# praateekmahajan/moving-mnist-vae

Measured on AMD Instinct MI355X. Metric: frames/sec/GPU VAE train step, 20×64×64 batch; ELBO vs CPU ref, higher is better.
Workload: dtype bf16; 1 GPU; BASELINE configs[1]: 256 clips x 20 frames x 64x64 per GPU per step (=5120 frames), conv-VAE z=128, Gaussian NLL sigma=0.1 + KL (normal_vae_1_kl_0_mmd), Adam, random-init weights, Bernoulli(0.0521) q=2 labels; parallelism=dp1, rccl_ranks=1, grad_exchange=none, bn=per-rank batch statistics

## Files before the change

moving-mnist-vae_amd/csrc/conv_fstream.hip:

```cpp
#include <hip/hip_runtime.h>

#include <stdlib.h>
#include <string.h>

#include "kernels.hpp"
#include "tile_common.hpp"

namespace mmvae {

struct Conv3StreamArgs {
  const void* x; const void* w; const void* wsc; void* y; void* ysc;
  const float* pro_scale; const float* pro_shift; int pro_relu;
  float* stats; float* stats_sc;
  const void* ym; const float* ms; const float* mb;
  int N, Ho, Hi;
  int HS, nunits;
};

template <int S, bool SC, bool PRO, bool BS = false>
__global__ __launch_bounds__(256, 2) void conv3_stream_kernel(Conv3StreamArgs a) {
  static_assert(!BS || (S == 1 && !SC && !PRO), "backward sums: the stride-1 data gradient");
  constexpr int KS = 3, PAD = 1, WO = 16, WI = S * WO, CB = 64;
  constexpr int WL = WI + 2;
  constexpr int ROWB = WL * CB;
  constexpr int NSLOT = KS + S;
  constexpr int WAVE_LDS = NSLOT * ROWB;
  constexpr int RV = S * WI * CB / 1024;
  constexpr int NPRIME = (KS - S + S - 1) / S;
  extern __shared__ __attribute__((aligned(16))) char smem[];
  const int t = threadIdx.x, lane = t & 63, wv = __builtin_amdgcn_readfirstlane(t >> 6), gq = lane >> 4, r = lane & 15;
  char* ring = smem + 2048 + wv * WAVE_LDS;
  for (int s = 0; s < NSLOT; ++s) {
    if (lane < 4) *reinterpret_cast<Vec16*>(ring + s * ROWB + lane * 16) = Vec16{{0, 0, 0, 0}};
    else if (lane < 8) *reinterpret_cast<Vec16*>(ring + s * ROWB + (WL - 1) * CB + (lane - 4) * 16) = Vec16{{0, 0, 0, 0}};
  }
  Vec16 wA[KS * KS][2], wS[2];
#pragma unroll
  for (int m = 0; m < 2; ++m) {
    const int c = 8 * (r >> 2) + 4 * m + (r & 3);
#pragma unroll
    for (int tap = 0; tap < KS * KS; ++tap)
      wA[tap][m] = *reinterpret_cast<const Vec16*>(reinterpret_cast<const char*>(a.w) + ((c * KS * KS + tap) * 32 + 8 * gq) * 2);
    wS[m] = SC ? *reinterpret_cast<const Vec16*>(reinterpret_cast<const char*>(a.wsc) + (c * 32 + 8 * gq) * 2) : Vec16{{0, 0, 0, 0}};
  }
  float psc[8], psh[8];
  if (PRO) {
    const int c = (lane & 3) * 8;
#pragma unroll
    for (int j = 0; j < 8; ++j) { psc[j] = a.pro_scale[c + j]; psh[j] = a.pro_shift[c + j]; }
  }
  const float lo = a.pro_relu ? 0.f : -__builtin_inff();
  float bms[8], bmb[8];
  if (BS) {
#pragma unroll
    for (int j = 0; j < 8; ++j) { bms[j] = a.ms[8 * gq + j]; bmb[j] = a.mb[8 * gq + j]; }
  }
  Vec16 yv = Vec16{{0, 0, 0, 0}};
  float st[SC ? 4 : 2][8];
#pragma unroll
  for (int q = 0; q < (SC ? 4 : 2); ++q)
#pragma unroll
    for (int j = 0; j < 8; ++j) st[q][j] = 0.f;

  const bf16_t* __restrict__ X = reinterpret_cast<const bf16_t*>(a.x);
  const int nblk = gridDim.x;
  int u_first, u_step, u_end;
  if ((nblk & 7) == 0) {
    const int per = (a.nunits + 7) >> 3;
    const int lo_u = (blockIdx.x & 7) * per;
    u_first = lo_u + (blockIdx.x >> 3) * 4 + wv; u_step = (nblk >> 3) * 4; u_end = min(a.nunits, lo_u + per);
  } else { u_first = blockIdx.x * 4 + wv; u_step = nblk * 4; u_end = a.nunits; }
  const int nstrips = a.Ho / a.HS;
  const int nq = a.HS + NPRIME;

  Vec16 xv[RV];
  auto issue = [&](int u, int q) {
    const int n = u / nstrips, oh0 = (u - n * nstrips) * a.HS;
    const int top = S * (oh0 + q - NPRIME) + 1;
#pragma unroll
    for (int k = 0; k < RV; ++k) {
      const int byte = (lane + 64 * k) * 16;
      const int rr = byte / (WI * CB), off = byte - rr * (WI * CB);
      const int row = top - S + 1 + rr;
      xv[k] = Vec16{{0, 0, 0, 0}};
      if (row >= 0 && row < a.Hi) xv[k] = *reinterpret_cast<const Vec16*>(reinterpret_cast<const char*>(X) + (((long)n * a.Hi + row) * WI) * CB + off);
    }
    if (BS && q >= NPRIME)
      yv = *reinterpret_cast<const Vec16*>(reinterpret_cast<const char*>(a.ym) + ((((long)n * a.Ho + oh0 + q - NPRIME) * WO + r) * 32 + 8 * gq) * 2);
  };
  auto commit = [&](int u, int q) {
    const int n = u / nstrips, oh0 = (u - n * nstrips) * a.HS;
    const int top = S * (oh0 + q - NPRIME) + 1;
#pragma unroll
    for (int k = 0; k < RV; ++k) {
      const int byte = (lane + 64 * k) * 16;
      const int rr = byte / (WI * CB), off = byte - rr * (WI * CB);
      const int row = top - S + 1 + rr;
      Vec16 v = xv[k];
      if (PRO && row >= 0 && row < a.Hi) {
        float f[8];
        Elem<bf16_t>::unpack(v, f);
#pragma unroll
        for (int j = 0; j < 8; ++j) f[j] = fmaxf(f[j] * psc[j] + psh[j], lo);
        v = Elem<bf16_t>::pack(f);
      }
      *reinterpret_cast<Vec16*>(ring + ((row + 4 * NSLOT) % NSLOT) * ROWB + CB + off) = v;
    }
    (void)n;
  };

  int u = u_first, q = 0;
  if (u < u_end) issue(u, 0);
  while (u < u_end) {
    commit(u, q);
    const Vec16 ycur = yv;
    int un = u, qn = q + 1;
    if (qn == nq) { un = u + u_step; qn = 0; }
    if (un < u_end) issue(un, qn);
    __builtin_amdgcn_sched_barrier(0);
    if (q >= NPRIME) {
      const int n = u / nstrips, oh = (u - n * nstrips) * a.HS + q - NPRIME;
      const int first = S * oh - PAD;
      f32x4 acc[2], asc[2];
#pragma unroll
      for (int m = 0; m < 2; ++m) { acc[m] = (f32x4){0, 0, 0, 0}; asc[m] = (f32x4){0, 0, 0, 0}; }
#pragma unroll
      for (int kh = 0; kh < KS; ++kh) {
        const char* rowp = ring + ((first + kh + 4 * NSLOT) % NSLOT) * ROWB;
#pragma unroll
        for (int kw = 0; kw < KS; ++kw) {
          const Vec16 b = *reinterpret_cast<const Vec16*>(rowp + (S * r + kw) * CB + gq * 16);
          acc[0] = mma_bf16(wA[kh * KS + kw][0], b, acc[0]);
          acc[1] = mma_bf16(wA[kh * KS + kw][1], b, acc[1]);
          if (SC && kh == 1 && kw == 1) { asc[0] = mma_bf16(wS[0], b, asc[0]); asc[1] = mma_bf16(wS[1], b, asc[1]); }
        }
      }
      const long po = (((long)n * a.Ho + oh) * WO + r) * 32 + 8 * gq;
      {
        const float v[8] = {acc[0][0], acc[0][1], acc[0][2], acc[0][3], acc[1][0], acc[1][1], acc[1][2], acc[1][3]};
        if constexpr (BS) {
          float ym[8], vr[8];
          Elem<bf16_t>::unpack(ycur, ym);
          Elem<bf16_t>::unpack(Elem<bf16_t>::pack(v), vr);
#pragma unroll
          for (int j = 0; j < 8; ++j) {
            const float g = (ym[j] * bms[j] + bmb[j] > 0.f) ? vr[j] : 0.f;
            st[0][j] += g; st[1][j] += g * ym[j];
          }
        } else {
#pragma unroll
          for (int j = 0; j < 8; ++j) { st[0][j] += v[j]; st[1][j] += v[j] * v[j]; }
        }
        dstore8<bf16_t>(reinterpret_cast<bf16_t*>(a.y) + po, v, false);
      }
      if constexpr (SC) {
        const float v[8] = {asc[0][0], asc[0][1], asc[0][2], asc[0][3], asc[1][0], asc[1][1], asc[1][2], asc[1][3]};
#pragma unroll
        for (int j = 0; j < 8; ++j) { st[2][j] += v[j]; st[3][j] += v[j] * v[j]; }
        dstore8<bf16_t>(reinterpret_cast<bf16_t*>(a.ysc) + po, v, false);
      }
    }
    __builtin_amdgcn_sched_barrier(0);
    u = un; q = qn;
  }
  float* sb = reinterpret_cast<float*>(smem);
#pragma unroll
  for (int qq = 0; qq < (SC ? 4 : 2); ++qq)
#pragma unroll
    for (int j = 0; j < 8; ++j) {
      const float v = row16_sum(st[qq][j]);
      if (r == 0) sb[wv * 128 + qq * 32 + 8 * gq + j] = v;
    }
  __syncthreads();
  if (t < (SC ? 128 : 64)) {
    const float v = (sb[t] + sb[128 + t]) + (sb[256 + t] + sb[384 + t]);
    float* dst = t < 64 ? a.stats : a.stats_sc;
    if (dst) dst[(long)blockIdx.x * 64 + (t & 63)] = v;
  }
}

bool conv3_stream_ok(int dt, int Cin, int Cout, int k, int s, int p, int Hin, int Win) {
  return dt == DT_BF16 && Cin == 32 && Cout == 32 && k == 3 && p == 1 && (s == 1 || s == 2) && Hin == Win && Win == 16 * s;
}

int launch_conv3_stream(int dt, int stride, const void* x, const void* w, const void* wsc, void* y, void* ysc, const float* pro_scale,
                        const float* pro_shift, int pro_relu, float* stats, float* stats_sc, int N, int Ho, hipStream_t s) {
  if (dt != DT_BF16 || (stride != 1 && stride != 2) || (wsc && stride != 2) || ((wsc != nullptr) != (ysc != nullptr))) {
    set_error("conv3_stream: bf16, stride 1 or 2, shortcut only with stride 2"); return MMVAE_ERR_UNSUPPORTED;
  }
  Conv3StreamArgs a; memset(&a, 0, sizeof(a));
  a.x = x; a.w = w; a.wsc = wsc; a.y = y; a.ysc = ysc; a.pro_scale = pro_scale; a.pro_shift = pro_shift; a.pro_relu = pro_relu;
  a.stats = stats; a.stats_sc = stats_sc; a.N = N; a.Ho = Ho; a.Hi = stride * Ho;
  a.HS = Ho % 8 == 0 ? 8 : Ho;
  a.nunits = N * (Ho / a.HS);
  int gx = stride == 1 ? 768 : 512;
  while (gx > 8 && (long)gx * 4 > a.nunits) gx -= 8;
  const bool pro = pro_scale != nullptr;
  const size_t lds = 2048 + 4 * (size_t)((3 + stride) * (stride * 16 + 2) * 64);
#define MMVAE_C3(S_, SC_, P_) hipLaunchKernelGGL((conv3_stream_kernel<S_, SC_, P_>), dim3(gx), dim3(256), lds, s, a)
  if (stride == 2) { if (wsc) { if (pro) MMVAE_C3(2, true, true); else MMVAE_C3(2, true, false); } else { if (pro) MMVAE_C3(2, false, true); else MMVAE_C3(2, false, false); } }
  else { if (pro) MMVAE_C3(1, false, true); else MMVAE_C3(1, false, false); }
#undef MMVAE_C3
  note_launch_bytes((double)N * 32 * 2.0 * ((double)a.Hi * a.Hi + (double)Ho * Ho * (wsc ? 2 : 1)));
  const int rc = check_launch("conv3_stream");
  return rc ? rc : gx;
}

int launch_conv3_stream_bwd(int dt, const void* dy, const void* w_flipped, void* dx, const void* ym, const float* ms, const float* mb, float* sums,
                            int N, int H, hipStream_t s) {
  if (dt != DT_BF16 || H != 16 || !ym || !ms || !mb || !sums) { set_error("conv3_stream_bwd: bf16, 16x16 maps, mask operand and sums required"); return MMVAE_ERR_UNSUPPORTED; }
  Conv3StreamArgs a; memset(&a, 0, sizeof(a));
  a.x = dy; a.w = w_flipped; a.y = dx; a.stats = sums; a.ym = ym; a.ms = ms; a.mb = mb; a.N = N; a.Ho = H; a.Hi = H;
  a.HS = 8; a.nunits = N * (H / a.HS);
  int gx = 768;
  while (gx > 8 && (long)gx * 4 > a.nunits) gx -= 8;
  const size_t lds = 2048 + 4 * (size_t)(4 * 18 * 64);
  hipLaunchKernelGGL((conv3_stream_kernel<1, false, false, true>), dim3(gx), dim3(256), lds, s, a);
  note_launch_bytes((double)N * 32 * 2.0 * 3.0 * H * H);
  const int rc = check_launch("conv3_stream_bwd");
  return rc ? rc : gx;
}

struct TailFwdStreamArgs {
  const void* y2; const void* ys; const float* s2; const float* b2; const float* ss; const float* bs;
  const float* w; const float* bias; float* r_raw; float* stats;
  int N, H, HS, nunits;
};

template <bool F8I>
__global__ __launch_bounds__(256, 2) void tail_fwd_stream_kernel(TailFwdStreamArgs a) {
  constexpr int KS = 3, W = 64, CB = 32;
  constexpr int NC = F8I ? 16 : 8;
  constexpr int WL = W + 2, ROWB = WL * CB, NSLOT = KS + 1, WAVE_LDS = NSLOT * ROWB, NPRIME = 2;
  extern __shared__ __attribute__((aligned(16))) char smem[];
  const int t = threadIdx.x, lane = t & 63, wv = __builtin_amdgcn_readfirstlane(t >> 6), gq = lane >> 4, r = lane & 15;
  char* ring = smem + 64 + wv * WAVE_LDS;
  for (int s = 0; s < NSLOT; ++s) {
    if (lane < 2) *reinterpret_cast<Vec16*>(ring + s * ROWB + lane * 16) = Vec16{{0, 0, 0, 0}};
    else if (lane < 4) *reinterpret_cast<Vec16*>(ring + s * ROWB + (WL - 1) * CB + (lane - 2) * 16) = Vec16{{0, 0, 0, 0}};
  }
  Vec16 wA[2];
  {
    float f0[8], f1[8];
#pragma unroll
    for (int j = 0; j < 8; ++j) {
      const int c = 8 * (gq & 1) + j;
      f0[j] = r < 3 ? a.w[c * 9 + (gq >> 1) * 3 + r] : 0.f;
      f1[j] = (r < 3 && gq < 2) ? a.w[c * 9 + 2 * 3 + r] : 0.f;
    }
    wA[0] = Elem<bf16_t>::pack(f0); wA[1] = Elem<bf16_t>::pack(f1);
  }
  const float bias = a.bias ? a.bias[0] : 0.f;
  float c2s[NC], c2b[NC], css[NC];
  {
    const int c = F8I ? 0 : (lane & 1) * 8;
#pragma unroll
    for (int j = 0; j < NC; ++j) { c2s[j] = a.s2[c + j]; c2b[j] = a.b2[c + j] + a.bs[c + j]; css[j] = a.ss[c + j]; }
  }
  float st1 = 0.f, st2 = 0.f;
  const int nblk = gridDim.x;
  int u_first, u_step, u_end;
  if ((nblk & 7) == 0) {
    const int per = (a.nunits + 7) >> 3;
    const int lo_u = (blockIdx.x & 7) * per;
    u_first = lo_u + (blockIdx.x >> 3) * 4 + wv; u_step = (nblk >> 3) * 4; u_end = min(a.nunits, lo_u + per);
  } else { u_first = blockIdx.x * 4 + wv; u_step = nblk * 4; u_end = a.nunits; }
  const int nstrips = a.H / a.HS;
  const int nq = a.HS + NPRIME;
  Vec16 v2[2], vs[2];
  auto issue = [&](int u, int q) {
    const int n = u / nstrips, oh0 = (u - n * nstrips) * a.HS;
    const int row = oh0 + q - NPRIME + 1;
#pragma unroll
    for (int k = 0; k < (F8I ? 1 : 2); ++k) {
      v2[k] = Vec16{{0, 0, 0, 0}}; vs[k] = Vec16{{0, 0, 0, 0}};
      if (row >= 0 && row < a.H) {
        const long off = (((long)n * a.H + row) * W) * (F8I ? 16 : CB) + (lane + 64 * k) * 16;
        v2[k] = *reinterpret_cast<const Vec16*>(reinterpret_cast<const char*>(a.y2) + off);
        vs[k] = *reinterpret_cast<const Vec16*>(reinterpret_cast<const char*>(a.ys) + off);
      }
    }
  };
  auto commit = [&](int u, int q) {
    const int n = u / nstrips, oh0 = (u - n * nstrips) * a.HS;
    const int row = oh0 + q - NPRIME + 1;
    const bool in = row >= 0 && row < a.H;
    if constexpr (F8I) {
      float f2[16], fs[16];
#pragma unroll
      for (int q4 = 0; q4 < 4; ++q4) { unpack4_fp8(v2[0].w[q4], f2 + 4 * q4); unpack4_fp8(vs[0].w[q4], fs + 4 * q4); }
#pragma unroll
      for (int j = 0; j < 16; ++j) f2[j] = in ? fmaxf(f2[j] * c2s[j] + c2b[j] + fs[j] * css[j], 0.f) : 0.f;
      char* dstp = ring + ((row + 4 * NSLOT) % NSLOT) * ROWB + CB + lane * 32;
      *reinterpret_cast<Vec16*>(dstp) = Elem<bf16_t>::pack(f2);
      *reinterpret_cast<Vec16*>(dstp + 16) = Elem<bf16_t>::pack(f2 + 8);
    } else {
#pragma unroll
      for (int k = 0; k < 2; ++k) {
        float f2[8], fs[8];
        Elem<bf16_t>::unpack(v2[k], f2);
        Elem<bf16_t>::unpack(vs[k], fs);
#pragma unroll
        for (int j = 0; j < 8; ++j) f2[j] = in ? fmaxf(f2[j] * c2s[j] + c2b[j] + fs[j] * css[j], 0.f) : 0.f;
        *reinterpret_cast<Vec16*>(ring + ((row + 4 * NSLOT) % NSLOT) * ROWB + CB + (lane + 64 * k) * 16) = Elem<bf16_t>::pack(f2);
      }
    }
    (void)n;
  };
  int u = u_first, q = 0;
  if (u < u_end) issue(u, 0);
  while (u < u_end) {
    commit(u, q);
    int un = u, qn = q + 1;
    if (qn == nq) { un = u + u_step; qn = 0; }
    if (un < u_end) issue(un, qn);
    __builtin_amdgcn_sched_barrier(0);
    if (q >= NPRIME) {
      const int n = u / nstrips, oh = (u - n * nstrips) * a.HS + q - NPRIME;
      const char* row01 = ring + ((oh - 1 + (gq >> 1) + 4 * NSLOT) % NSLOT) * ROWB;
      const char* row2 = ring + ((oh + 1 + 4 * NSLOT) % NSLOT) * ROWB;
      float d0[4], d1[4], d2[4];
#pragma unroll
      for (int pt = 0; pt < 4; ++pt) {
        const int po = (16 * pt + r + 1) * CB + (gq & 1) * 16;
        f32x4 acc = mma_bf16(wA[0], *reinterpret_cast<const Vec16*>(row01 + po), (f32x4){0, 0, 0, 0});
        acc = mma_bf16(wA[1], *reinterpret_cast<const Vec16*>(row2 + po), acc);
        d0[pt] = acc[0]; d1[pt] = acc[1]; d2[pt] = acc[2];
        asm volatile("" : "+v"(d0[pt]), "+v"(d1[pt]), "+v"(d2[pt]));
      }
      float outv[4];
#pragma unroll
      for (int pt = 0; pt < 4; ++pt) {
        float left = __builtin_bit_cast(float, __builtin_amdgcn_mov_dpp(__builtin_bit_cast(int, d0[pt]), 0x111, 0xf, 0xf, true));
        if (pt > 0) {
          const float pl = __builtin_bit_cast(float, __builtin_amdgcn_mov_dpp(__builtin_bit_cast(int, d0[pt - 1]), 0x121, 0xf, 0xf, true));
          left = r == 0 ? pl : left;
        }
        float right = __builtin_bit_cast(float, __builtin_amdgcn_mov_dpp(__builtin_bit_cast(int, d2[pt]), 0x101, 0xf, 0xf, true));
        if (pt < 3) {
          const float nr = __builtin_bit_cast(float, __builtin_amdgcn_mov_dpp(__builtin_bit_cast(int, d2[pt + 1]), 0x12f, 0xf, 0xf, true));
          right = r == 15 ? nr : right;
        }
        outv[pt] = (left + d1[pt]) + right + bias;
      }
      if (gq == 0) {
        float* orow = a.r_raw + ((long)n * a.H + oh) * W + r;
#pragma unroll
        for (int pt = 0; pt < 4; ++pt) {
          orow[16 * pt] = outv[pt];
          st1 += outv[pt]; st2 += outv[pt] * outv[pt];
        }
      }
    }
    __builtin_amdgcn_sched_barrier(0);
    u = un; q = qn;
  }
  st1 = row16_sum(st1); st2 = row16_sum(st2);
  float* sb = reinterpret_cast<float*>(smem);
  if (lane == 0) { sb[wv * 2] = st1; sb[wv * 2 + 1] = st2; }
  __syncthreads();
  if (a.stats && t < 2) a.stats[(long)blockIdx.x * 2 + t] = (sb[t] + sb[2 + t]) + (sb[4 + t] + sb[6 + t]);
}

struct ConvT4StreamArgs {
  const void* x; const void* w; void* y;
  const float* pro_scale; const float* pro_shift; int pro_relu;
  float* stats;
  int N, Hi, HS, nunits;
};

template <int WIN, bool PRO, bool F8O = false>
__global__ __launch_bounds__(256, 3) void convT4_stream_kernel(ConvT4StreamArgs a) {
  constexpr int CB = 32, WL = WIN + 2, ROWB = WL * CB, NSLOT = 4, NPRIME = 2;
  constexpr int CBO = F8O ? 16 : 32;
  constexpr int OROWB = 2 * WIN * CBO;
  constexpr int WAVE_LDS = NSLOT * ROWB + OROWB;
  constexpr int XV = (WIN * CB + 1023) / 1024;
  constexpr int NPT = WIN / 16;
  extern __shared__ __attribute__((aligned(16))) char smem[];
  const int t = threadIdx.x, lane = t & 63, wv = __builtin_amdgcn_readfirstlane(t >> 6), gq = lane >> 4, r = lane & 15;
  char* ring = smem + 1024 + wv * WAVE_LDS;
  char* orow = ring + NSLOT * ROWB;
  for (int s = 0; s < NSLOT; ++s) {
    if (lane < 2) *reinterpret_cast<Vec16*>(ring + s * ROWB + lane * 16) = Vec16{{0, 0, 0, 0}};
    else if (lane < 4) *reinterpret_cast<Vec16*>(ring + s * ROWB + (WL - 1) * CB + (lane - 2) * 16) = Vec16{{0, 0, 0, 0}};
  }
  Vec16 wA[4][2];
#pragma unroll
  for (int p = 0; p < 4; ++p)
#pragma unroll
    for (int th = 0; th < 2; ++th)
      wA[p][th] = *reinterpret_cast<const Vec16*>(reinterpret_cast<const char*>(a.w) + p * 2048 + r * 128 + th * 64 + gq * 16);
  const int dwl[2] = {(gq >> 1) ? -1 : 0, (gq >> 1) ? 0 : 1};
  float psc[8], psh[8];
  if (PRO) {
    const int c = (lane & 1) * 8;
#pragma unroll
    for (int j = 0; j < 8; ++j) { psc[j] = a.pro_scale[c + j]; psh[j] = a.pro_shift[c + j]; }
  }
  const float lo = a.pro_relu ? 0.f : -__builtin_inff();
  float st1[4] = {0, 0, 0, 0}, st2[4] = {0, 0, 0, 0};
  const int nblk = gridDim.x;
  int u_first, u_step, u_end;
  if ((nblk & 7) == 0) {
    const int per = (a.nunits + 7) >> 3;
    const int lo_u = (blockIdx.x & 7) * per;
    u_first = lo_u + (blockIdx.x >> 3) * 4 + wv; u_step = (nblk >> 3) * 4; u_end = min(a.nunits, lo_u + per);
  } else { u_first = blockIdx.x * 4 + wv; u_step = nblk * 4; u_end = a.nunits; }
  const int nstrips = a.Hi / a.HS;
  const int nq = a.HS + NPRIME;
  const bool xlane = lane * 16 < WIN * CB;
  Vec16 xv = Vec16{{0, 0, 0, 0}};
  auto issue = [&](int u, int q) {
    const int n = u / nstrips, q0 = (u - n * nstrips) * a.HS;
    const int row = q0 + q - NPRIME + 1;
    xv = Vec16{{0, 0, 0, 0}};
    if (xlane && row >= 0 && row < a.Hi) xv = *reinterpret_cast<const Vec16*>(reinterpret_cast<const char*>(a.x) + (((long)n * a.Hi + row) * WIN) * CB + lane * 16);
  };
  auto commit = [&](int u, int q) {
    const int n = u / nstrips, q0 = (u - n * nstrips) * a.HS;
    const int row = q0 + q - NPRIME + 1;
    if (xlane) {
      Vec16 v = xv;
      if (PRO && row >= 0 && row < a.Hi) {
        float f[8];
        Elem<bf16_t>::unpack(v, f);
#pragma unroll
        for (int j = 0; j < 8; ++j) f[j] = fmaxf(f[j] * psc[j] + psh[j], lo);
        v = Elem<bf16_t>::pack(f);
      }
      *reinterpret_cast<Vec16*>(ring + ((row + 4 * NSLOT) % NSLOT) * ROWB + CB + lane * 16) = v;
    }
    (void)n; (void)XV;
  };
  int u = u_first, q = 0;
  if (u < u_end) issue(u, 0);
  while (u < u_end) {
    commit(u, q);
    int un = u, qn = q + 1;
    if (qn == nq) { un = u + u_step; qn = 0; }
    if (un < u_end) issue(un, qn);
    __builtin_amdgcn_sched_barrier(0);
    if (q >= NPRIME) {
      const int n = u / nstrips, iq = (u - n * nstrips) * a.HS + q - NPRIME;
#pragma unroll
      for (int ph = 0; ph < 2; ++ph) {
#pragma unroll
        for (int pw = 0; pw < 2; ++pw) {
          f32x4 acc[NPT];
#pragma unroll
          for (int pt = 0; pt < NPT; ++pt) acc[pt] = (f32x4){0, 0, 0, 0};
#pragma unroll
          for (int th = 0; th < 2; ++th) {
            const int dh = ph == 0 ? (th == 0 ? 0 : -1) : (th == 0 ? 1 : 0);
            const char* rowp = ring + ((iq + dh + 4 * NSLOT) % NSLOT) * ROWB;
#pragma unroll
            for (int pt = 0; pt < NPT; ++pt) {
              const Vec16 b = *reinterpret_cast<const Vec16*>(rowp + (16 * pt + r + dwl[pw] + 1) * CB + (gq & 1) * 16);
              acc[pt] = mma_bf16(wA[2 * ph + pw][th], b, acc[pt]);
            }
          }
#pragma unroll
          for (int pt = 0; pt < NPT; ++pt) {
#pragma unroll
            for (int j = 0; j < 4; ++j) { st1[j] += acc[pt][j]; st2[j] += acc[pt][j] * acc[pt][j]; }
            if constexpr (F8O) {
              *reinterpret_cast<uint32_t*>(orow + (2 * (16 * pt + r) + pw) * CBO + gq * 4) = pack4_fp8(acc[pt][0], acc[pt][1], acc[pt][2], acc[pt][3]);
            } else {
              uint2 o;
              o.x = pack2_bf16(acc[pt][0], acc[pt][1]); o.y = pack2_bf16(acc[pt][2], acc[pt][3]);
              *reinterpret_cast<uint2*>(orow + (2 * (16 * pt + r) + pw) * CB + gq * 8) = o;
            }
          }
        }
        asm volatile("" ::: "memory");
        char* dst = reinterpret_cast<char*>(a.y) + (((long)n * (2 * a.Hi) + 2 * iq + ph) * (2 * WIN)) * CBO;
#pragma unroll
        for (int k = 0; k < OROWB / 1024; ++k) *reinterpret_cast<Vec16*>(dst + (lane + 64 * k) * 16) = *reinterpret_cast<const Vec16*>(orow + (lane + 64 * k) * 16);
      }
    }
    __builtin_amdgcn_sched_barrier(0);
    u = un; q = qn;
  }
  float* sb = reinterpret_cast<float*>(smem);
#pragma unroll
  for (int j = 0; j < 4; ++j) {
    const float v1 = row16_sum(st1[j]), v2 = row16_sum(st2[j]);
    if (r == 0) { sb[wv * 32 + 4 * gq + j] = v1; sb[wv * 32 + 16 + 4 * gq + j] = v2; }
  }
  __syncthreads();
  if (a.stats && t < 32) a.stats[(long)blockIdx.x * 32 + t] = (sb[t] + sb[32 + t]) + (sb[64 + t] + sb[96 + t]);
}

struct Up5TailFwdArgs {
  const void* y1; const float* p1s; const float* p1b; const void* w2;
  const void* xin; const float* pxs; const float* pxb; const void* wu;
  const float* s2; const float* b2; const float* ss; const float* bs;
  const float* w; const float* bias; float* r_raw; float* stats;
  int N, HS, nunits;
};

template <bool PRO_X>
__global__ __launch_bounds__(256, 2) void up5_tail_fwd_kernel(Up5TailFwdArgs a) {
  constexpr int WIN = 32, Hi = 32, W = 64, H = 64, CB = 32;
  constexpr int IWL = WIN + 2, IROWB = IWL * CB, NSLOT = 4;
  constexpr int JWL = W + 2, JROWB = JWL * CB;
  constexpr int WAVE_LDS = 2 * NSLOT * IROWB + NSLOT * JROWB;
  extern __shared__ __attribute__((aligned(16))) char smem[];
  const int t = threadIdx.x, lane = t & 63, wv = __builtin_amdgcn_readfirstlane(t >> 6), gq = lane >> 4, r = lane & 15;
  char* ringA = smem + 64 + wv * WAVE_LDS;
  char* ringX = ringA + NSLOT * IROWB;
  char* ringJ = ringX + NSLOT * IROWB;
  for (int sl = 0; sl < NSLOT; ++sl) {
    if (lane < 2) { *reinterpret_cast<Vec16*>(ringA + sl * IROWB + lane * 16) = Vec16{{0, 0, 0, 0}}; *reinterpret_cast<Vec16*>(ringX + sl * IROWB + lane * 16) = Vec16{{0, 0, 0, 0}}; }
    else if (lane < 4) { *reinterpret_cast<Vec16*>(ringA + sl * IROWB + (IWL - 1) * CB + (lane - 2) * 16) = Vec16{{0, 0, 0, 0}}; *reinterpret_cast<Vec16*>(ringX + sl * IROWB + (IWL - 1) * CB + (lane - 2) * 16) = Vec16{{0, 0, 0, 0}}; }
    else if (lane < 6) *reinterpret_cast<Vec16*>(ringJ + sl * JROWB + (lane - 4) * 16) = Vec16{{0, 0, 0, 0}};
    else if (lane < 8) *reinterpret_cast<Vec16*>(ringJ + sl * JROWB + (JWL - 1) * CB + (lane - 6) * 16) = Vec16{{0, 0, 0, 0}};
  }
  Vec16 w2A[4][2], wuA[4][2];
#pragma unroll
  for (int p = 0; p < 4; ++p)
#pragma unroll
    for (int th = 0; th < 2; ++th) {
      w2A[p][th] = *reinterpret_cast<const Vec16*>(reinterpret_cast<const char*>(a.w2) + p * 2048 + r * 128 + th * 64 + gq * 16);
      wuA[p][th] = *reinterpret_cast<const Vec16*>(reinterpret_cast<const char*>(a.wu) + p * 2048 + r * 128 + th * 64 + gq * 16);
    }
  const int dwl[2] = {(gq >> 1) ? -1 : 0, (gq >> 1) ? 0 : 1};
  Vec16 wT[2];
  {
    float f0[8], f1[8];
#pragma unroll
    for (int j = 0; j < 8; ++j) {
      const int c = 8 * (gq & 1) + j;
      f0[j] = r < 3 ? a.w[c * 9 + (gq >> 1) * 3 + r] : 0.f;
      f1[j] = (r < 3 && gq < 2) ? a.w[c * 9 + 2 * 3 + r] : 0.f;
    }
    wT[0] = Elem<bf16_t>::pack(f0); wT[1] = Elem<bf16_t>::pack(f1);
  }
  const float bias = a.bias ? a.bias[0] : 0.f;
  float p1s[8], p1b[8], pxs[8], pxb[8];
  {
    const int c = (lane & 1) * 8;
#pragma unroll
    for (int j = 0; j < 8; ++j) { p1s[j] = a.p1s[c + j]; p1b[j] = a.p1b[c + j]; pxs[j] = PRO_X ? a.pxs[c + j] : 1.f; pxb[j] = PRO_X ? a.pxb[c + j] : 0.f; }
  }
  float js2[4], jb[4], jss[4];
#pragma unroll
  for (int j = 0; j < 4; ++j) { const int c = 4 * gq + j; js2[j] = a.s2[c]; jb[j] = a.b2[c] + a.bs[c]; jss[j] = a.ss[c]; }
  float st1 = 0.f, st2 = 0.f;
  const int nblk = gridDim.x;
  int u_first, u_step, u_end;
  if ((nblk & 7) == 0) {
    const int per = (a.nunits + 7) >> 3;
    const int lo_u = (blockIdx.x & 7) * per;
    u_first = lo_u + (blockIdx.x >> 3) * 4 + wv; u_step = (nblk >> 3) * 4; u_end = min(a.nunits, lo_u + per);
  } else { u_first = blockIdx.x * 4 + wv; u_step = nblk * 4; u_end = a.nunits; }
  const int nstrips = Hi / a.HS;
  constexpr int NPRIME = 2;
  const int nq = a.HS + 2 + NPRIME;
  Vec16 va = Vec16{{0, 0, 0, 0}}, vx = Vec16{{0, 0, 0, 0}};
  auto issue = [&](int u, int q) {
    const int n = u / nstrips, q0 = (u - n * nstrips) * a.HS;
    const int row = q0 - 1 + q - NPRIME + 1;
    va = Vec16{{0, 0, 0, 0}}; vx = Vec16{{0, 0, 0, 0}};
    if (row >= 0 && row < Hi) {
      const long off = (((long)n * Hi + row) * WIN) * CB + lane * 16;
      va = *reinterpret_cast<const Vec16*>(reinterpret_cast<const char*>(a.y1) + off);
      vx = *reinterpret_cast<const Vec16*>(reinterpret_cast<const char*>(a.xin) + off);
    }
  };
  auto commit = [&](int u, int q) {
    const int n = u / nstrips, q0 = (u - n * nstrips) * a.HS;
    const int row = q0 - 1 + q - NPRIME + 1;
    Vec16 ca = va, cx = vx;
    if (row >= 0 && row < Hi) {
      float f[8];
      Elem<bf16_t>::unpack(ca, f);
#pragma unroll
      for (int j = 0; j < 8; ++j) f[j] = fmaxf(f[j] * p1s[j] + p1b[j], 0.f);
      ca = Elem<bf16_t>::pack(f);
      if (PRO_X) {
        Elem<bf16_t>::unpack(cx, f);
#pragma unroll
        for (int j = 0; j < 8; ++j) f[j] = fmaxf(f[j] * pxs[j] + pxb[j], 0.f);
        cx = Elem<bf16_t>::pack(f);
      }
    }
    const int slot = (row + 4 * NSLOT) % NSLOT;
    *reinterpret_cast<Vec16*>(ringA + slot * IROWB + CB + lane * 16) = ca;
    *reinterpret_cast<Vec16*>(ringX + slot * IROWB + CB + lane * 16) = cx;
    (void)n;
  };
  int u = u_first, q = 0;
  if (u < u_end) issue(u, 0);
  while (u < u_end) {
    commit(u, q);
    int un = u, qn = q + 1;
    if (qn == nq) { un = u + u_step; qn = 0; }
    if (un < u_end) issue(un, qn);
    __builtin_amdgcn_sched_barrier(0);
    if (q >= NPRIME) {
      const int n = u / nstrips, q0 = (u - n * nstrips) * a.HS;
      const int iq = q0 - 1 + q - NPRIME;
      const bool inside = iq >= 0 && iq < Hi;
#pragma unroll
      for (int ph = 0; ph < 2; ++ph) {
        char* jrow = ringJ + ((2 * iq + ph + 8 * NSLOT) % NSLOT) * JROWB;
        if (!inside) {
          for (int i = lane; i < (W * CB) / 16; i += 64) *reinterpret_cast<Vec16*>(jrow + CB + i * 16) = Vec16{{0, 0, 0, 0}};
          continue;
        }
#pragma unroll
        for (int pw = 0; pw < 2; ++pw) {
          f32x4 acc2[2], accS[2];
#pragma unroll
          for (int pt = 0; pt < 2; ++pt) { acc2[pt] = (f32x4){0, 0, 0, 0}; accS[pt] = (f32x4){0, 0, 0, 0}; }
#pragma unroll
          for (int th = 0; th < 2; ++th) {
            const int dh = ph == 0 ? (th == 0 ? 0 : -1) : (th == 0 ? 1 : 0);
            const int sl = (iq + dh + 4 * NSLOT) % NSLOT;
#pragma unroll
            for (int pt = 0; pt < 2; ++pt) {
              const int off = sl * IROWB + (16 * pt + r + dwl[pw] + 1) * CB + (gq & 1) * 16;
              acc2[pt] = mma_bf16(w2A[2 * ph + pw][th], *reinterpret_cast<const Vec16*>(ringA + off), acc2[pt]);
              accS[pt] = mma_bf16(wuA[2 * ph + pw][th], *reinterpret_cast<const Vec16*>(ringX + off), accS[pt]);
            }
          }
#pragma unroll
          for (int pt = 0; pt < 2; ++pt) {
            float o[4];
#pragma unroll
            for (int j = 0; j < 4; ++j) o[j] = fmaxf(acc2[pt][j] * js2[j] + jb[j] + accS[pt][j] * jss[j], 0.f);
            *reinterpret_cast<uint2*>(jrow + (1 + 2 * (16 * pt + r) + pw) * CB + gq * 8) = make_uint2(pack2_bf16(o[0], o[1]), pack2_bf16(o[2], o[3]));
          }
        }
      }
      asm volatile("" ::: "memory");
#pragma unroll
      for (int k = 0; k < 2; ++k) {
        const int oh = 2 * iq - 1 + k;
        if (oh < 2 * q0 || oh >= 2 * (q0 + a.HS) || oh < 0 || oh >= H) continue;
        f32x4 acc[4];
        const char* row01 = ringJ + ((oh - 1 + (gq >> 1) + 8 * NSLOT) % NSLOT) * JROWB;
        const char* row2 = ringJ + ((oh + 1 + 8 * NSLOT) % NSLOT) * JROWB;
#pragma unroll
        for (int pt = 0; pt < 4; ++pt) {
          const int po = (16 * pt + r + 1) * CB + (gq & 1) * 16;
          acc[pt] = mma_bf16(wT[0], *reinterpret_cast<const Vec16*>(row01 + po), (f32x4){0, 0, 0, 0});
          acc[pt] = mma_bf16(wT[1], *reinterpret_cast<const Vec16*>(row2 + po), acc[pt]);
        }
        float d0[4], d1[4], d2[4];
#pragma unroll
        for (int pt = 0; pt < 4; ++pt) {
          d0[pt] = acc[pt][0]; d1[pt] = acc[pt][1]; d2[pt] = acc[pt][2];
          asm volatile("" : "+v"(d0[pt]), "+v"(d1[pt]), "+v"(d2[pt]));
        }
        float outv[4];
#pragma unroll
        for (int pt = 0; pt < 4; ++pt) {
          float left = __builtin_bit_cast(float, __builtin_amdgcn_mov_dpp(__builtin_bit_cast(int, d0[pt]), 0x111, 0xf, 0xf, true));
          if (pt > 0) {
            const float pl = __builtin_bit_cast(float, __builtin_amdgcn_mov_dpp(__builtin_bit_cast(int, d0[pt - 1]), 0x121, 0xf, 0xf, true));
            left = r == 0 ? pl : left;
          }
          float right = __builtin_bit_cast(float, __builtin_amdgcn_mov_dpp(__builtin_bit_cast(int, d2[pt]), 0x101, 0xf, 0xf, true));
          if (pt < 3) {
            const float nr = __builtin_bit_cast(float, __builtin_amdgcn_mov_dpp(__builtin_bit_cast(int, d2[pt + 1]), 0x12f, 0xf, 0xf, true));
            right = r == 15 ? nr : right;
          }
          outv[pt] = (left + d1[pt]) + right + bias;
        }
        if (gq == 0) {
          float* orow = a.r_raw + ((long)n * H + oh) * W + r;
#pragma unroll
          for (int pt = 0; pt < 4; ++pt) {
            orow[16 * pt] = outv[pt];
            st1 += outv[pt]; st2 += outv[pt] * outv[pt];
          }
        }
      }
    }
    __builtin_amdgcn_sched_barrier(0);
    u = un; q = qn;
  }
  st1 = row16_sum(st1); st2 = row16_sum(st2);
  float* sb = reinterpret_cast<float*>(smem);
  if (lane == 0) { sb[wv * 2] = st1; sb[wv * 2 + 1] = st2; }
  __syncthreads();
  if (a.stats && t < 2) a.stats[(long)blockIdx.x * 2 + t] = (sb[t] + sb[2 + t]) + (sb[4 + t] + sb[6 + t]);
}

bool up5_tail_fwd_ok(int dt, int OC, int C, int Cin, int Hin, int Hout) {
  return dt == DT_BF16 && OC == 1 && C == 16 && Cin == 16 && Hin == 32 && Hout == 64;
}
int launch_up5_tail_fwd(const void* y1, const float* p1s, const float* p1b, const void* w2_up, const void* xin, const float* pxs, const float* pxb,
                        const void* wu_up, const float* s2, const float* b2, const float* ss, const float* bs, const float* w, const float* bias,
                        float* r_raw, float* stats, int N, hipStream_t s) {
  Up5TailFwdArgs a; memset(&a, 0, sizeof(a));
  a.y1 = y1; a.p1s = p1s; a.p1b = p1b; a.w2 = w2_up; a.xin = xin; a.pxs = pxs; a.pxb = pxb; a.wu = wu_up;
  a.s2 = s2; a.b2 = b2; a.ss = ss; a.bs = bs; a.w = w; a.bias = bias; a.r_raw = r_raw; a.stats = stats;
  a.N = N; a.HS = 16; a.nunits = N * (32 / a.HS);
  int gx = 512;
  while (gx > 1 && (long)gx * 4 > a.nunits) gx -= gx > 8 ? 8 : 1;
  const size_t lds = 64 + 4 * (size_t)(2 * 4 * 34 * 32 + 4 * 66 * 32);
  static bool attr_set = false;
  if (!attr_set) {
    hipError_t e = hipFuncSetAttribute(reinterpret_cast<const void*>(&up5_tail_fwd_kernel<false>), hipFuncAttributeMaxDynamicSharedMemorySize, 160 * 1024);
    if (e == hipSuccess) e = hipFuncSetAttribute(reinterpret_cast<const void*>(&up5_tail_fwd_kernel<true>), hipFuncAttributeMaxDynamicSharedMemorySize, 160 * 1024);
    if (e != hipSuccess) { set_error("up5_tail_fwd: hipFuncSetAttribute: %s", hipGetErrorString(e)); return MMVAE_ERR_HIP; }
    attr_set = true;
  }
  if (pxs) hipLaunchKernelGGL(up5_tail_fwd_kernel<true>, dim3(gx), dim3(256), lds, s, a);
  else hipLaunchKernelGGL(up5_tail_fwd_kernel<false>, dim3(gx), dim3(256), lds, s, a);
  note_launch_bytes((double)N * (2.0 * 32 * 32 * 16 * 2 + 64 * 64 * 4.0));
  const int rc = check_launch("up5_tail_fwd");
  return rc ? rc : gx;
}

bool convT4_stream_ok(int dt, int Cin, int Cout, int k, int s, int p, int Hin, int Win) {
  return dt == DT_BF16 && Cin == 16 && Cout == 16 && k == 4 && s == 2 && p == 1 && Hin == Win && (Win == 32 || Win == 16);
}
int launch_convT4_stream(int dt, const void* x, const void* w_up, void* y, const float* pro_scale, const float* pro_shift, int pro_relu, float* stats,
                         int N, int Hin, hipStream_t s, int f8out) {
  if (!convT4_stream_ok(dt, 16, 16, 4, 2, 1, Hin, Hin)) { set_error("convT4_stream: bf16, 16 -> 16 channels, k4 s2 p1, 16x16 or 32x32 input"); return MMVAE_ERR_UNSUPPORTED; }
  ConvT4StreamArgs a; memset(&a, 0, sizeof(a));
  a.x = x; a.w = w_up; a.y = y; a.pro_scale = pro_scale; a.pro_shift = pro_shift; a.pro_relu = pro_relu; a.stats = stats;
  a.N = N; a.Hi = Hin; a.HS = Hin % 8 == 0 ? 8 : Hin; a.nunits = N * (Hin / a.HS);
  int gx = Hin == 32 ? 1024 : 768;
  while (gx > 8 && (long)gx * 4 > a.nunits) gx -= 8;
  const bool pro = pro_scale != nullptr;
  const size_t lds = 1024 + 4 * (size_t)(4 * (Hin + 2) * 32 + 2 * Hin * 32);
  if (f8out && Hin != 32) { set_error("convT4_stream: e4m3 output only for the 32x32 -> 64x64 layers"); return MMVAE_ERR_UNSUPPORTED; }
  if (f8out) { if (pro) hipLaunchKernelGGL((convT4_stream_kernel<32, true, true>), dim3(gx), dim3(256), lds, s, a); else hipLaunchKernelGGL((convT4_stream_kernel<32, false, true>), dim3(gx), dim3(256), lds, s, a); }
  else if (Hin == 32) { if (pro) hipLaunchKernelGGL((convT4_stream_kernel<32, true>), dim3(gx), dim3(256), lds, s, a); else hipLaunchKernelGGL((convT4_stream_kernel<32, false>), dim3(gx), dim3(256), lds, s, a); }
  else { if (pro) hipLaunchKernelGGL((convT4_stream_kernel<16, true>), dim3(gx), dim3(256), lds, s, a); else hipLaunchKernelGGL((convT4_stream_kernel<16, false>), dim3(gx), dim3(256), lds, s, a); }
  note_launch_bytes((double)N * 16 * (2.0 + (f8out ? 4.0 : 8.0)) * Hin * Hin);
  const int rc = check_launch("convT4_stream");
  return rc ? rc : gx;
}

bool tail_fwd_stream_ok(int dt, int OC, int H, int W) {
  return dt == DT_BF16 && OC == 1 && W == 64 && H == 64;
}
int launch_tail_fwd_stream(int dt, const void* y2, const float* s2, const float* b2, const void* ys, const float* ss, const float* bs, const float* w,
                           const float* bias, float* r_raw, float* stats, int N, int H, int W, hipStream_t s, int f8in) {
  if (!tail_fwd_stream_ok(dt, 1, H, W)) { set_error("tail_fwd_stream: bf16, one output plane, 64x64"); return MMVAE_ERR_UNSUPPORTED; }
  TailFwdStreamArgs a; memset(&a, 0, sizeof(a));
  a.y2 = y2; a.ys = ys; a.s2 = s2; a.b2 = b2; a.ss = ss; a.bs = bs; a.w = w; a.bias = bias; a.r_raw = r_raw; a.stats = stats;
  a.N = N; a.H = H; a.HS = 16; a.nunits = N * (H / a.HS);
  int gx = 768;
  while (gx > 1 && (long)gx * 4 > a.nunits) gx -= gx > 8 ? 8 : 1;
  const size_t lds = 64 + 4 * (size_t)(4 * 66 * 32);
  if (f8in) hipLaunchKernelGGL(tail_fwd_stream_kernel<true>, dim3(gx), dim3(256), lds, s, a);
  else hipLaunchKernelGGL(tail_fwd_stream_kernel<false>, dim3(gx), dim3(256), lds, s, a);
  note_launch_bytes((double)N * H * W * (2 * 16 * (f8in ? 1.0 : 2.0) + 4.0));
  const int rc = check_launch("tail_fwd_stream");
  return rc ? rc : gx;
}

}
```

Before: 849,100 frames/s.

## Keep up5 tail input rows in registers via DPP shifts instead of LDS rings

Removes the per-wave LDS ring buffers for the transposed-conv inputs (y1 and skip) in the fused up5 tail kernel. Each lane now loads its own column pixels directly, applies the BN/ReLU prologue on packed bf16, and builds the left and right shifted neighbours with DPP lane moves into a two-row register window that feeds the MFMAs. The loop is unrolled by two so the register window alternates, and the priming depth drops from two rows to one. This cuts LDS traffic and LDS footprint, possibly improving occupancy, but raises VGPR pressure and adds DPP and select work.

```diff
diff --git a/moving-mnist-vae_amd/csrc/conv_fstream.hip b/moving-mnist-vae_amd/csrc/conv_fstream.hip
--- a/moving-mnist-vae_amd/csrc/conv_fstream.hip
+++ b/moving-mnist-vae_amd/csrc/conv_fstream.hip
@@ -500,22 +500,39 @@
   int N, HS, nunits;
 };
 
+__device__ __forceinline__ u32x4_t up5_prologue(u32x4_t v, const float* sc, const float* sh) {
+  u32x4_t o;
+#pragma unroll
+  for (int i = 0; i < 4; ++i) {
+    const float lo = fmaxf(fmaf(__uint_as_float(v[i] << 16), sc[2 * i], sh[2 * i]), 0.f);
+    const float hi = fmaxf(fmaf(__uint_as_float(v[i] & 0xffff0000u), sc[2 * i + 1], sh[2 * i + 1]), 0.f);
+    o[i] = pack2_bf16(lo, hi);
+  }
+  return o;
+}
+__device__ __forceinline__ float up5_join(float y2, float s2, float b, float ys, float ss) {
+#pragma clang fp contract(off)
+  return fmaxf(y2 * s2 + b + ys * ss, 0.f);
+}
+__device__ __forceinline__ float up5_sqacc(float acc, float v) {
+#pragma clang fp contract(off)
+  return acc + v * v;
+}
+__device__ __forceinline__ f32x4 up5_mma(const Vec16& a, u32x4_t b, f32x4 c) {
+  return __builtin_amdgcn_mfma_f32_16x16x32_bf16(__builtin_bit_cast(bf16x8, a), __builtin_bit_cast(bf16x8, b), c, 0, 0, 0);
+}
+
 template <bool PRO_X>
 __global__ __launch_bounds__(256, 2) void up5_tail_fwd_kernel(Up5TailFwdArgs a) {
   constexpr int WIN = 32, Hi = 32, W = 64, H = 64, CB = 32;
-  constexpr int IWL = WIN + 2, IROWB = IWL * CB, NSLOT = 4;
-  constexpr int JWL = W + 2, JROWB = JWL * CB;
-  constexpr int WAVE_LDS = 2 * NSLOT * IROWB + NSLOT * JROWB;
+  constexpr int NSLOT = 4, JWL = W + 2, JROWB = JWL * CB;
+  constexpr int WAVE_LDS = NSLOT * JROWB;
   extern __shared__ __attribute__((aligned(16))) char smem[];
   const int t = threadIdx.x, lane = t & 63, wv = __builtin_amdgcn_readfirstlane(t >> 6), gq = lane >> 4, r = lane & 15;
-  char* ringA = smem + 64 + wv * WAVE_LDS;
-  char* ringX = ringA + NSLOT * IROWB;
-  char* ringJ = ringX + NSLOT * IROWB;
+  char* ringJ = smem + 64 + wv * WAVE_LDS;
   for (int sl = 0; sl < NSLOT; ++sl) {
-    if (lane < 2) { *reinterpret_cast<Vec16*>(ringA + sl * IROWB + lane * 16) = Vec16{{0, 0, 0, 0}}; *reinterpret_cast<Vec16*>(ringX + sl * IROWB + lane * 16) = Vec16{{0, 0, 0, 0}}; }
-    else if (lane < 4) { *reinterpret_cast<Vec16*>(ringA + sl * IROWB + (IWL - 1) * CB + (lane - 2) * 16) = Vec16{{0, 0, 0, 0}}; *reinterpret_cast<Vec16*>(ringX + sl * IROWB + (IWL - 1) * CB + (lane - 2) * 16) = Vec16{{0, 0, 0, 0}}; }
-    else if (lane < 6) *reinterpret_cast<Vec16*>(ringJ + sl * JROWB + (lane - 4) * 16) = Vec16{{0, 0, 0, 0}};
-    else if (lane < 8) *reinterpret_cast<Vec16*>(ringJ + sl * JROWB + (JWL - 1) * CB + (lane - 6) * 16) = Vec16{{0, 0, 0, 0}};
+    if (lane < 2) *reinterpret_cast<Vec16*>(ringJ + sl * JROWB + lane * 16) = Vec16{{0, 0, 0, 0}};
+    else if (lane < 4) *reinterpret_cast<Vec16*>(ringJ + sl * JROWB + (JWL - 1) * CB + (lane - 2) * 16) = Vec16{{0, 0, 0, 0}};
   }
   Vec16 w2A[4][2], wuA[4][2];
 #pragma unroll
@@ -525,7 +542,6 @@
       w2A[p][th] = *reinterpret_cast<const Vec16*>(reinterpret_cast<const char*>(a.w2) + p * 2048 + r * 128 + th * 64 + gq * 16);
       wuA[p][th] = *reinterpret_cast<const Vec16*>(reinterpret_cast<const char*>(a.wu) + p * 2048 + r * 128 + th * 64 + gq * 16);
     }
-  const int dwl[2] = {(gq >> 1) ? -1 : 0, (gq >> 1) ? 0 : 1};
   Vec16 wT[2];
   {
     float f0[8], f1[8];
@@ -540,7 +556,7 @@
   const float bias = a.bias ? a.bias[0] : 0.f;
   float p1s[8], p1b[8], pxs[8], pxb[8];
   {
-    const int c = (lane & 1) * 8;
+    const int c = (gq & 1) * 8;
 #pragma unroll
     for (int j = 0; j < 8; ++j) { p1s[j] = a.p1s[c + j]; p1b[j] = a.p1b[c + j]; pxs[j] = PRO_X ? a.pxs[c + j] : 1.f; pxb[j] = PRO_X ? a.pxb[c + j] : 0.f; }
   }
@@ -556,132 +572,151 @@
     u_first = lo_u + (blockIdx.x >> 3) * 4 + wv; u_step = (nblk >> 3) * 4; u_end = min(a.nunits, lo_u + per);
   } else { u_first = blockIdx.x * 4 + wv; u_step = nblk * 4; u_end = a.nunits; }
   const int nstrips = Hi / a.HS;
-  constexpr int NPRIME = 2;
-  const int nq = a.HS + 2 + NPRIME;
-  Vec16 va = Vec16{{0, 0, 0, 0}}, vx = Vec16{{0, 0, 0, 0}};
+  const int nq = a.HS + 2;
+  const bool look_l = gq >= 2, look_r = gq < 2;
+  const bool fix_l = look_l && r == 0, fix_r = look_r && r == 15;
+  u32x4_t ra[2], rx[2];
+  u32x4_t wa[2][4], wx[2][4];
+#pragma unroll
+  for (int f = 0; f < 4; ++f) {
+    ra[f >> 1] = (u32x4_t){0, 0, 0, 0}; rx[f >> 1] = (u32x4_t){0, 0, 0, 0};
+    wa[0][f] = (u32x4_t){0, 0, 0, 0}; wa[1][f] = (u32x4_t){0, 0, 0, 0}; wx[0][f] = (u32x4_t){0, 0, 0, 0}; wx[1][f] = (u32x4_t){0, 0, 0, 0};
+  }
   auto issue = [&](int u, int q) {
     const int n = u / nstrips, q0 = (u - n * nstrips) * a.HS;
-    const int row = q0 - 1 + q - NPRIME + 1;
-    va = Vec16{{0, 0, 0, 0}}; vx = Vec16{{0, 0, 0, 0}};
+    const int row = q0 - 1 + q;
+    ra[0] = (u32x4_t){0, 0, 0, 0}; ra[1] = (u32x4_t){0, 0, 0, 0}; rx[0] = (u32x4_t){0, 0, 0, 0}; rx[1] = (u32x4_t){0, 0, 0, 0};
     if (row >= 0 && row < Hi) {
-      const long off = (((long)n * Hi + row) * WIN) * CB + lane * 16;
-      va = *reinterpret_cast<const Vec16*>(reinterpret_cast<const char*>(a.y1) + off);
-      vx = *reinterpret_cast<const Vec16*>(reinterpret_cast<const char*>(a.xin) + off);
+      const long off = (((long)n * Hi + row) * WIN + r) * CB + (gq & 1) * 16;
+#pragma unroll
+      for (int pt = 0; pt < 2; ++pt) {
+        ra[pt] = *reinterpret_cast<const u32x4_t*>(reinterpret_cast<const char*>(a.y1) + off + pt * 16 * CB);
+        rx[pt] = *reinterpret_cast<const u32x4_t*>(reinterpret_cast<const char*>(a.xin) + off + pt * 16 * CB);
+      }
     }
   };
-  auto commit = [&](int u, int q) {
-    const int n = u / nstrips, q0 = (u - n * nstrips) * a.HS;
-    const int row = q0 - 1 + q - NPRIME + 1;
-    Vec16 ca = va, cx = vx;
-    if (row >= 0 && row < Hi) {
-      float f[8];
-      Elem<bf16_t>::unpack(ca, f);
-#pragma unroll
-      for (int j = 0; j < 8; ++j) f[j] = fmaxf(f[j] * p1s[j] + p1b[j], 0.f);
-      ca = Elem<bf16_t>::pack(f);
-      if (PRO_X) {
-        Elem<bf16_t>::unpack(cx, f);
-#pragma unroll
-        for (int j = 0; j < 8; ++j) f[j] = fmaxf(f[j] * pxs[j] + pxb[j], 0.f);
-        cx = Elem<bf16_t>::pack(f);
-      }
-    }
-    const int slot = (row + 4 * NSLOT) % NSLOT;
-    *reinterpret_cast<Vec16*>(ringA + slot * IROWB + CB + lane * 16) = ca;
-    *reinterpret_cast<Vec16*>(ringX + slot * IROWB + CB + lane * 16) = cx;
-    (void)n;
+  auto spread = [&](const u32x4_t* c, u32x4_t* w) {
+#pragma unroll
+    for (int i = 0; i < 4; ++i) {
+      const int c0 = (int)c[0][i], c1 = (int)c[1][i];
+      const int l0 = __builtin_amdgcn_update_dpp(c0, c0, 0x111, 0xc, 0xf, true);
+      int l1 = __builtin_amdgcn_update_dpp(c1, c1, 0x111, 0xc, 0xf, true);
+      const int c0_15 = __builtin_amdgcn_mov_dpp(c0, 0x121, 0xf, 0xf, true);
+      l1 = fix_l ? c0_15 : l1;
+      int r0 = __builtin_amdgcn_update_dpp(c0, c0, 0x101, 0x3, 0xf, true);
+      const int r1 = __builtin_amdgcn_update_dpp(c1, c1, 0x101, 0x3, 0xf, true);
+      const int c1_0 = __builtin_amdgcn_mov_dpp(c1, 0x12f, 0xf, 0xf, true);
+      r0 = fix_r ? c1_0 : r0;
+      w[0][i] = (uint32_t)l0; w[1][i] = (uint32_t)r0; w[2][i] = (uint32_t)l1; w[3][i] = (uint32_t)r1;
+    }
   };
   int u = u_first, q = 0;
   if (u < u_end) issue(u, 0);
   while (u < u_end) {
-    commit(u, q);
-    int un = u, qn = q + 1;
-    if (qn == nq) { un = u + u_step; qn = 0; }
-    if (un < u_end) issue(un, qn);
-    __builtin_amdgcn_sched_barrier(0);
-    if (q >= NPRIME) {
-      const int n = u / nstrips, q0 = (u - n * nstrips) * a.HS;
-      const int iq = q0 - 1 + q - NPRIME;
-      const bool inside = iq >= 0 && iq < Hi;
-#pragma unroll
-      for (int ph = 0; ph < 2; ++ph) {
-        char* jrow = ringJ + ((2 * iq + ph + 8 * NSLOT) % NSLOT) * JROWB;
-        if (!inside) {
-          for (int i = lane; i < (W * CB) / 16; i += 64) *reinterpret_cast<Vec16*>(jrow + CB + i * 16) = Vec16{{0, 0, 0, 0}};
-          continue;
-        }
-#pragma unroll
-        for (int pw = 0; pw < 2; ++pw) {
-          f32x4 acc2[2], accS[2];
-#pragma unroll
-          for (int pt = 0; pt < 2; ++pt) { acc2[pt] = (f32x4){0, 0, 0, 0}; accS[pt] = (f32x4){0, 0, 0, 0}; }
-#pragma unroll
-          for (int th = 0; th < 2; ++th) {
-            const int dh = ph == 0 ? (th == 0 ? 0 : -1) : (th == 0 ? 1 : 0);
-            const int sl = (iq + dh + 4 * NSLOT) % NSLOT;
+#pragma unroll
+    for (int s2 = 0; s2 < 2; ++s2) {
+      if (u >= u_end) break;
+      {
+        const int n = u / nstrips, q0 = (u - n * nstrips) * a.HS;
+        const int row = q0 - 1 + q;
+        const bool rok = row >= 0 && row < Hi;
+        (void)n;
+        u32x4_t ca[2], cx[2];
+#pragma unroll
+        for (int pt = 0; pt < 2; ++pt) {
+          const u32x4_t pa = up5_prologue(ra[pt], p1s, p1b);
+          const u32x4_t px = PRO_X ? up5_prologue(rx[pt], pxs, pxb) : rx[pt];
+          ca[pt] = rok ? pa : (u32x4_t){0, 0, 0, 0};
+          cx[pt] = rok ? px : (u32x4_t){0, 0, 0, 0};
+        }
+        spread(ca, wa[s2]);
+        spread(cx, wx[s2]);
+      }
+      int un = u, qn = q + 1;
+      if (qn == nq) { un = u + u_step; qn = 0; }
+      if (un < u_end) issue(un, qn);
+      __builtin_amdgcn_sched_barrier(0);
+      if (q >= 1) {
+        const int n = u / nstrips, q0 = (u - n * nstrips) * a.HS;
+        const int R = q0 - 1 + q;
+#pragma unroll
+        for (int ph = 1; ph >= 0; --ph) {
+          const int jr = 2 * R - ph;
+          char* jrow = ringJ + ((jr + 8 * NSLOT) % NSLOT) * JROWB;
+          if (jr < 0 || jr >= H) {
+            for (int i = lane; i < (W * CB) / 16; i += 64) *reinterpret_cast<Vec16*>(jrow + CB + i * 16) = Vec16{{0, 0, 0, 0}};
+            continue;
+          }
+#pragma unroll
+          for (int pw = 0; pw < 2; ++pw) {
+            f32x4 acc2[2], accS[2];
+#pragma unroll
+            for (int pt = 0; pt < 2; ++pt) { acc2[pt] = (f32x4){0, 0, 0, 0}; accS[pt] = (f32x4){0, 0, 0, 0}; }
+#pragma unroll
+            for (int th = 0; th < 2; ++th) {
+              const int sl = th == 0 ? s2 : s2 ^ 1;
+#pragma unroll
+              for (int pt = 0; pt < 2; ++pt) {
+                acc2[pt] = up5_mma(w2A[2 * ph + pw][th], wa[sl][2 * pt + pw], acc2[pt]);
+                accS[pt] = up5_mma(wuA[2 * ph + pw][th], wx[sl][2 * pt + pw], accS[pt]);
+              }
+            }
 #pragma unroll
             for (int pt = 0; pt < 2; ++pt) {
-              const int off = sl * IROWB + (16 * pt + r + dwl[pw] + 1) * CB + (gq & 1) * 16;
-              acc2[pt] = mma_bf16(w2A[2 * ph + pw][th], *reinterpret_cast<const Vec16*>(ringA + off), acc2[pt]);
-              accS[pt] = mma_bf16(wuA[2 * ph + pw][th], *reinterpret_cast<const Vec16*>(ringX + off), accS[pt]);
+              float o[4];
+#pragma unroll
+              for (int j = 0; j < 4; ++j) o[j] = up5_join(acc2[pt][j], js2[j], jb[j], accS[pt][j], jss[j]);
+              *reinterpret_cast<uint2*>(jrow + (1 + 2 * (16 * pt + r) + pw) * CB + gq * 8) = make_uint2(pack2_bf16(o[0], o[1]), pack2_bf16(o[2], o[3]));
             }
           }
-#pragma unroll
-          for (int pt = 0; pt < 2; ++pt) {
-            float o[4];
-#pragma unroll
-            for (int j = 0; j < 4; ++j) o[j] = fmaxf(acc2[pt][j] * js2[j] + jb[j] + accS[pt][j] * jss[j], 0.f);
-            *reinterpret_cast<uint2*>(jrow + (1 + 2 * (16 * pt + r) + pw) * CB + gq * 8) = make_uint2(pack2_bf16(o[0], o[1]), pack2_bf16(o[2], o[3]));
-          }
-        }
-      }
-      asm volatile("" ::: "memory");
-#pragma unroll
-      for (int k = 0; k < 2; ++k) {
-        const int oh = 2 * iq - 1 + k;
-        if (oh < 2 * q0 || oh >= 2 * (q0 + a.HS) || oh < 0 || oh >= H) continue;
-        f32x4 acc[4];
-        const char* row01 = ringJ + ((oh - 1 + (gq >> 1) + 8 * NSLOT) % NSLOT) * JROWB;
-        const char* row2 = ringJ + ((oh + 1 + 8 * NSLOT) % NSLOT) * JROWB;
-#pragma unroll
-        for (int pt = 0; pt < 4; ++pt) {
-          const int po = (16 * pt + r + 1) * CB + (gq & 1) * 16;
-          acc[pt] = mma_bf16(wT[0], *reinterpret_cast<const Vec16*>(row01 + po), (f32x4){0, 0, 0, 0});
-          acc[pt] = mma_bf16(wT[1], *reinterpret_cast<const Vec16*>(row2 + po), acc[pt]);
-        }
-        float d0[4], d1[4], d2[4];
-#pragma unroll
-        for (int pt = 0; pt < 4; ++pt) {
-          d0[pt] = acc[pt][0]; d1[pt] = acc[pt][1]; d2[pt] = acc[pt][2];
-          asm volatile("" : "+v"(d0[pt]), "+v"(d1[pt]), "+v"(d2[pt]));
-        }
-        float outv[4];
-#pragma unroll
-        for (int pt = 0; pt < 4; ++pt) {
-          float left = __builtin_bit_cast(float, __builtin_amdgcn_mov_dpp(__builtin_bit_cast(int, d0[pt]), 0x111, 0xf, 0xf, true));
-          if (pt > 0) {
-            const float pl = __builtin_bit_cast(float, __builtin_amdgcn_mov_dpp(__builtin_bit_cast(int, d0[pt - 1]), 0x121, 0xf, 0xf, true));
-            left = r == 0 ? pl : left;
-          }
-          float right = __builtin_bit_cast(float, __builtin_amdgcn_mov_dpp(__builtin_bit_cast(int, d2[pt]), 0x101, 0xf, 0xf, true));
-          if (pt < 3) {
-            const float nr = __builtin_bit_cast(float, __builtin_amdgcn_mov_dpp(__builtin_bit_cast(int, d2[pt + 1]), 0x12f, 0xf, 0xf, true));
-            right = r == 15 ? nr : right;
-          }
-          outv[pt] = (left + d1[pt]) + right + bias;
-        }
-        if (gq == 0) {
-          float* orow = a.r_raw + ((long)n * H + oh) * W + r;
+        }
+        asm volatile("" ::: "memory");
+#pragma unroll
+        for (int k = 0; k < 2; ++k) {
+          const int oh = 2 * R - 2 + k;
+          if (oh < 2 * q0 || oh >= 2 * (q0 + a.HS) || oh < 0 || oh >= H) continue;
+          f32x4 acc[4];
+          const char* row01 = ringJ + ((oh - 1 + (gq >> 1) + 8 * NSLOT) % NSLOT) * JROWB;
+          const char* row2 = ringJ + ((oh + 1 + 8 * NSLOT) % NSLOT) * JROWB;
 #pragma unroll
           for (int pt = 0; pt < 4; ++pt) {
-            orow[16 * pt] = outv[pt];
-            st1 += outv[pt]; st2 += outv[pt] * outv[pt];
-          }
-        }
-      }
-    }
-    __builtin_amdgcn_sched_barrier(0);
-    u = un; q = qn;
+            const int po = (16 * pt + r + 1) * CB + (gq & 1) * 16;
+            acc[pt] = mma_bf16(wT[0], *reinterpret_cast<const Vec16*>(row01 + po), (f32x4){0, 0, 0, 0});
+            acc[pt] = mma_bf16(wT[1], *reinterpret_cast<const Vec16*>(row2 + po), acc[pt]);
+          }
+          float d0[4], d1[4], d2[4];
+#pragma unroll
+          for (int pt = 0; pt < 4; ++pt) {
+            d0[pt] = acc[pt][0]; d1[pt] = acc[pt][1]; d2[pt] = acc[pt][2];
+            asm volatile("" : "+v"(d0[pt]), "+v"(d1[pt]), "+v"(d2[pt]));
+          }
+          float outv[4];
+#pragma unroll
+          for (int pt = 0; pt < 4; ++pt) {
+            float left = __builtin_bit_cast(float, __builtin_amdgcn_mov_dpp(__builtin_bit_cast(int, d0[pt]), 0x111, 0xf, 0xf, true));
+            if (pt > 0) {
+              const float pl = __builtin_bit_cast(float, __builtin_amdgcn_mov_dpp(__builtin_bit_cast(int, d0[pt - 1]), 0x121, 0xf, 0xf, true));
+              left = r == 0 ? pl : left;
+            }
+            float right = __builtin_bit_cast(float, __builtin_amdgcn_mov_dpp(__builtin_bit_cast(int, d2[pt]), 0x101, 0xf, 0xf, true));
+            if (pt < 3) {
+              const float nr = __builtin_bit_cast(float, __builtin_amdgcn_mov_dpp(__builtin_bit_cast(int, d2[pt + 1]), 0x12f, 0xf, 0xf, true));
+              right = r == 15 ? nr : right;
+            }
+            outv[pt] = (left + d1[pt]) + right + bias;
+          }
+          if (gq == 0) {
+            float* orow = a.r_raw + ((long)n * H + oh) * W + r;
+#pragma unroll
+            for (int pt = 0; pt < 4; ++pt) {
+              orow[16 * pt] = outv[pt];
+              st1 += outv[pt]; st2 = up5_sqacc(st2, outv[pt]);
+            }
+          }
+        }
+      }
+      u = un; q = qn;
+    }
   }
   st1 = row16_sum(st1); st2 = row16_sum(st2);
   float* sb = reinterpret_cast<float*>(smem);
@@ -702,7 +737,7 @@
   a.N = N; a.HS = 16; a.nunits = N * (32 / a.HS);
   int gx = 512;
   while (gx > 1 && (long)gx * 4 > a.nunits) gx -= gx > 8 ? 8 : 1;
-  const size_t lds = 64 + 4 * (size_t)(2 * 4 * 34 * 32 + 4 * 66 * 32);
+  const size_t lds = 64 + 4 * (size_t)(4 * 66 * 32);
   static bool attr_set = false;
   if (!attr_set) {
     hipError_t e = hipFuncSetAttribute(reinterpret_cast<const void*>(&up5_tail_fwd_kernel<false>), hipFuncAttributeMaxDynamicSharedMemorySize, 160 * 1024);
```

Result: no change. 853,300 frames/s, median of 6 (+0.5%).
